# Black-Phoenix/CUDA-SfM

Hardware: AMD Instinct MI355X
Metric: RANSAC E-matrix hypotheses/sec (8-point, fused scoring), inlier-mask parity vs CPU oracle (higher is better)
Workload: dtype f32

## Files before the change

### cuda-sfm_amd/csrc/abi.hip

```cpp
#include "common.hpp"
#include "buffer_ranges.hpp"
#include "device_math.hpp"
#include "fuse_math.hpp"
#include "chain_adjust_math.hpp"
#include "ring_math.hpp"
#include <stdarg.h>
#include <stdio.h>
#include <string.h>
#include <new>
#include <atomic>
#include <vector>
#include <algorithm>
#include <initializer_list>

namespace sfm {

static thread_local char g_err[512] = "";

void set_error(const char *fmt, ...)
{
    va_list ap;
    va_start(ap, fmt);
    vsnprintf(g_err, sizeof(g_err), fmt, ap);
    va_end(ap);
// ... 494 lines not shown

int sfm_extract_sift(sfm_ctx *ctx, sfm_sift_point *d_sift, int max_pts, const float *d_image, int width, int height,
                     int pitch, int num_octaves, double init_blur, float thresh, float lowest_scale, int scale_up,
                     float *d_temp, int *num_pts, int *num_stored)
{
    SFM_REQUIRE(ctx && d_sift && d_image && num_pts, SFM_E_INVALID, "null argument");
    SFM_REQUIRE(width > 0 && height > 0 && width <= 16384 && height <= 16384 && pitch >= width, SFM_E_INVALID,
                "image %d x %d pitch %d", width, height, pitch);
    SFM_REQUIRE(num_octaves >= 1 && num_octaves <= 7, SFM_E_INVALID, "num_octaves %d outside 1..7", num_octaves);
    SFM_REQUIRE(max_pts > 0, SFM_E_INVALID, "max_pts %d", max_pts);
    *num_pts = 0;
    if (num_stored) *num_stored = 0;
    SFM_HIP_TRY(hipSetDevice(ctx->device));
    return launch_extract_sift(ctx, d_sift, max_pts, d_image, width, height, pitch, num_octaves, init_blur, thresh, lowest_scale,
                               scale_up ? 1 : 0, d_temp, num_pts, num_stored);
}

int sfm_extract_sift_begin(sfm_ctx *ctx, sfm_sift_point *d_sift, int max_pts, const float *d_image, int width, int height,
                           int pitch, int num_octaves, double init_blur, float thresh, float lowest_scale, int scale_up, float *d_temp)
{
    SFM_REQUIRE(ctx && d_sift && d_image, SFM_E_INVALID, "null argument");
    SFM_REQUIRE(width > 0 && height > 0 && width <= 16384 && height <= 16384 && pitch >= width, SFM_E_INVALID,
                "image %d x %d pitch %d", width, height, pitch);
    SFM_REQUIRE(num_octaves >= 1 && num_octaves <= 7, SFM_E_INVALID, "num_octaves %d outside 1..7", num_octaves);
    SFM_REQUIRE(max_pts > 0, SFM_E_INVALID, "max_pts %d", max_pts);
    SFM_HIP_TRY(hipSetDevice(ctx->device));
    return launch_extract_sift_begin(ctx, d_sift, max_pts, d_image, width, height, pitch, num_octaves, init_blur, thresh, lowest_scale,
                                     scale_up ? 1 : 0, d_temp);
}

int sfm_extract_sift_end(sfm_ctx *ctx, int *num_pts, int *num_stored)
{
    SFM_REQUIRE(ctx && num_pts, SFM_E_INVALID, "null argument");
    *num_pts = 0;
    if (num_stored) *num_stored = 0;
    SFM_HIP_TRY(hipSetDevice(ctx->device));
    return launch_extract_sift_end(ctx, num_pts, num_stored);
}

int sfm_find_homography(sfm_ctx *ctx, const sfm_sift_point *d_sift, int num_pts, float h_H[9], int *num_matches,
                        int num_loops, float min_score, float max_ambiguity, float thresh, uint32_t seed,
                        const int32_t *h_pts, int32_t *h_counts, float *h_homo)
{
    SFM_REQUIRE(ctx && h_H && num_matches, SFM_E_INVALID, "null argument");
    *num_matches = 0;
    for (int i = 0; i < 9; ++i) h_H[i] = (i % 4 == 0) ? 1.0f : 0.0f;
    if (!d_sift || num_pts < 8 || num_loops <= 0) return SFM_OK;
    SFM_HIP_TRY(hipSetDevice(ctx->device));
    const int L = round_up(num_loops, 16);
    if (h_pts) {
        for (size_t i = 0; i < (size_t)4 * L; ++i)
            SFM_REQUIRE(h_pts[i] >= 0 && h_pts[i] < num_pts, SFM_E_INVALID, "sample index %d out of range", h_pts[i]);
    }
    int num_valid = 0;
    return launch_homography(ctx, d_sift, num_pts, h_pts, L, thresh, min_score, max_ambiguity, seed, &num_valid, h_H, num_matches, h_counts, h_homo);
}

int sfm_pair_create(sfm_ctx *ctx, const float h_K[9], const float h_Kinv[9], int image_count, int num_points, sfm_pair **out)
{
    SFM_REQUIRE(out, SFM_E_INVALID, "null out pointer");
    *out = nullptr;
    SFM_REQUIRE(ctx && h_K && h_Kinv, SFM_E_INVALID, "null argument");
    SFM_REQUIRE(image_count == 2, SFM_E_INVALID, "image_count must be 2 (the reference only ever uses two views, sfm.h:31)");
    SFM_REQUIRE(num_points > 0, SFM_E_INVALID, "num_points must be positive");
    SFM_HIP_TRY(hipSetDevice(ctx->device));
    sfm_pair *p = new (std::nothrow) sfm_pair();
    SFM_REQUIRE(p, SFM_E_NOMEM, "host allocation failed");
    p->ctx = ctx;
    p->holds_ctx_ref = true; ctx->refs++;
    p->image_count = image_count;
    p->n = num_points;
    p->cap_points = num_points;
    p->ld = round_up(num_points, 128);
    memcpy(p->h_Kinv, h_Kinv, sizeof(p->h_Kinv));
    int rc = SFM_OK;
    auto A = [&](auto **ptr, size_t count) { if (rc == SFM_OK) rc = dev_alloc(ptr, count); };
    A(&p->d_K, 9); A(&p->d_Kinv, 9);
    for (int i = 0; i < 2; ++i) { A(&p->d_U[i], (size_t)3 * p->ld); A(&p->d_X[i], (size_t)3 * p->ld); }
    A(&p->d_pts4, (size_t)p->ld);
    A(&p->d_E, 9); A(&p->d_P, 64); A(&p->d_Pinv, 64); A(&p->d_Pind, 8);
    A(&p->d_points, (size_t)4 * num_points);
    A(&p->d_mask, (size_t)num_points);
    A(&p->slot[0].key, 2); A(&p->d_best, 2); A(&p->d_clk, kClkWords); A(&p->d_bound, 10);
    if (rc != SFM_OK) { sfm_pair_destroy(p); return rc; }
    hipError_t e = hipMemcpyAsync(p->d_K, h_K, 9 * sizeof(float), hipMemcpyHostToDevice, ctx->stream);
    if (e == hipSuccess) e = hipMemcpyAsync(p->d_Kinv, h_Kinv, 9 * sizeof(float), hipMemcpyHostToDevice, ctx->stream);
    if (e == hipSuccess) e = hipMemsetAsync(p->slot[0].key, 0, 2 * sizeof(unsigned long long), ctx->stream);
    p->state.key_clean = true;
    if (e == hipSuccess) e = hipMemsetAsync(p->d_best, 0, 2 * sizeof(uint32_t), ctx->stream);
    if (e == hipSuccess) e = hipMemsetAsync(p->d_bound, 0, 10 * sizeof(unsigned long long), ctx->stream);
    if (e == hipSuccess) e = hipMemsetAsync(p->d_clk, 0, kClkWords * sizeof(unsigned long long), ctx->stream);
    if (e == hipSuccess) e = hipMemsetAsync(p->d_Pind, 0, 8 * sizeof(int), ctx->stream);
    if (e == hipSuccess) e = hipStreamSynchronize(ctx->stream);
    if (e != hipSuccess) { sfm_pair_destroy(p); set_error("pair init failed: %s", hipGetErrorString(e)); return SFM_E_HIP; }
    *out = p;
    return SFM_OK;
}

int sfm_pair_reset(sfm_pair *pair, int num_points)
{
    SFM_REQUIRE(pair, SFM_E_INVALID, "null pair");
    SFM_FLUSH(pair);
    SFM_REQUIRE(num_points > 0 && num_points <= pair->cap_points, SFM_E_INVALID,
                "num_points %d outside (0, %d] (the size the pair was created with)", num_points, pair->cap_points);
    pair->n = num_points;
    pair->ld = round_up(num_points, 128);
    pair->state.reset();
    return SFM_OK;
}

int sfm_pair_destroy(sfm_pair *p)
{
    if (!p) return SFM_OK;
    if (p->ctx) { (void)hipSetDevice(p->ctx->device); (void)hipStreamSynchronize(p->ctx->stream); }
    void *bufs[] = { p->d_K, p->d_Kinv, p->d_U[0], p->d_U[1], p->d_X[0], p->d_X[1], p->d_pts4, p->d_E, p->d_P, p->d_Pinv, p->d_Pind,
                     p->d_points, p->d_mask, p->d_best, p->d_clk, p->d_bound, p->d_cells, p->d_pts4s, p->d_tile_boxes, p->d_buckets,
                     p->d_rstate, p->d_rpoints, p->d_rreproj, p->d_rwork, p->d_vstate, p->d_vreproj, p->d_vwork, p->d_vhyp, p->d_vcounts, p->d_awork,
                     p->d_lwork, p->d_lhyp };
    for (void *b : bufs) if (b) (void)hipFree(b);
    for (ShardSlot &s : p->slot) shard_slot_free(s);
    if (p->pipe_stream) { (void)hipStreamSynchronize(p->pipe_stream); (void)hipStreamDestroy(p->pipe_stream); }
    for (hipEvent_t e : p->pipe_final) if (e) (void)hipEventDestroy(e);
    if (p->pipe_call) (void)hipEventDestroy(p->pipe_call);
    if (p->cells_ev) (void)hipEventDestroy(p->cells_ev);
    if (p->pipe_keys) (void)hipFree(p->pipe_keys);
    sfm_ctx *owner = p->holds_ctx_ref ? p->ctx : nullptr;
    delete p;
    ctx_release(owner);
    return SFM_OK;
}

int sfm_fill_xu(sfm_pair *pair, const sfm_sift_point *d_data)
{
    SFM_REQUIRE(pair && d_data, SFM_E_INVALID, "null argument");
    SFM_FLUSH(pair);
    SFM_HIP_TRY(hipSetDevice(pair->ctx->device));
    const int rc = launch_fill_xu(pair, d_data);
    if (rc == SFM_OK) pair->state.points_filled(unit_z_Kinv(pair->h_Kinv));
    return rc;
}

int sfm_set_points(sfm_pair *pair, const float *d_X0, const float *d_X1)
{
    SFM_REQUIRE(pair && d_X0 && d_X1, SFM_E_INVALID, "null argument");
    SFM_FLUSH(pair);
    SFM_HIP_TRY(hipSetDevice(pair->ctx->device));
    const int rc = launch_set_points(pair, d_X0, d_X1);
    if (rc == SFM_OK) pair->state.points_set();
    return rc;
}

void sfm_ransac_default_params(sfm_ransac_params *p, int num_points)
{
    if (!p) return;
    memset(p, 0, sizeof(*p));
    p->num_hypotheses = num_points >= 8 ? (uint32_t)(num_points / 8) : 1u;
    p->seed = 0x5EED5F3Du;
    p->threshold = 1e-6f;
    p->jacobi_sweeps = 0;
    p->kernel = SFM_KERNEL_AUTO;
}

int sfm_ransac_permutation_indices(sfm_ctx *ctx, int num_points, uint32_t seed, int32_t *d_indices)
{
    SFM_REQUIRE(ctx && d_indices, SFM_E_INVALID, "null argument");
    SFM_REQUIRE(num_points >= 8, SFM_E_INVALID, "need at least 8 points");
    SFM_HIP_TRY(hipSetDevice(ctx->device));
    return launch_permutation_indices(ctx, num_points, seed, d_indices);
}

static int score_shard(sfm_pair *pair, const sfm_ransac_params *p, uint64_t *d_key_out, const float *d_E)
{
    uint32_t h0, count;
    int rc = resolve_shard(pair, p, &h0, &count);
    if (rc != SFM_OK) return rc;
    SFM_FLUSH(pair);
    SFM_HIP_TRY(hipSetDevice(pair->ctx->device));
    return launch_ransac_score(pair, pair->slot[0], pair->ctx->stream, *p, h0, count, reinterpret_cast<unsigned long long *>(d_key_out), d_E);
}

int sfm_ransac_score(sfm_pair *pair, const sfm_ransac_params *p) { return score_shard(pair, p, nullptr, nullptr); }

int sfm_ransac_score_candidates(sfm_pair *pair, const sfm_ransac_params *p, const float *d_E)
{
    SFM_REQUIRE(d_E, SFM_E_INVALID, "null candidate pointer");
    return score_shard(pair, p, nullptr, d_E);
}

int sfm_ransac_score_into(sfm_pair *pair, const sfm_ransac_params *p, uint64_t *d_key_out)
{
    SFM_REQUIRE(d_key_out, SFM_E_INVALID, "null key pointer");
    return score_shard(pair, p, d_key_out, nullptr);
}

int sfm_ransac_score_into_slot(sfm_pair *pair, const sfm_ransac_params *p, uint64_t *d_key_out, int slot, void *hip_stream)
{
    SFM_REQUIRE(d_key_out, SFM_E_INVALID, "null key pointer");
    SFM_REQUIRE(slot == 0 || slot == 1, SFM_E_INVALID, "slot must be 0 or 1");
    uint32_t h0, count;
// ... 1376 lines not shown
```

### cuda-sfm_amd/csrc/common.hpp

```cpp
#pragma once
#include <hip/hip_runtime.h>
#include <stdint.h>
#include <stddef.h>
#include <string>
#include <atomic>
#include <type_traits>
#include "../../include/sfm_amd.h"
#include "pair_state.hpp"
#include "job_order.hpp"
#if SFM_AB
#include "../../include/sfm_amd_ab.h"
#endif

#if SFM_AB
#define SFM_SW(p, i) ((p).reserved[i])
#else
#define SFM_SW(p, i) 0
#endif

namespace sfm {

void set_error(const char *fmt, ...);

#define SFM_HIP_TRY(expr)                                                                      \
    do {                                                                                       \
        hipError_t err__ = (expr);                                                             \
        if (err__ != hipSuccess) {                                                             \
            ::sfm::set_error("%s failed: %s (%s:%d)", #expr, hipGetErrorString(err__), __FILE__, __LINE__); \
            return err__ == hipErrorOutOfMemory ? SFM_E_NOMEM : SFM_E_HIP;                     \
        }                                                                                      \
    } while (0)

#define SFM_REQUIRE(cond, code, ...)                                                           \
    do {                                                                                       \
        if (!(cond)) { ::sfm::set_error(__VA_ARGS__); return (code); }                         \
    } while (0)

#define SFM_FLUSH(pair)                                                                        \
    do { if ((pair)->pipe_pending) { const int rcf__ = sfm_pair_flush(pair); if (rcf__ != SFM_OK) return rcf__; } } while (0)

#define SFM_NEED(pair, stages)                                                                 \
    SFM_REQUIRE((pair)->state.has(stages), SFM_E_STATE, "%s", ::sfm::pair_stage_hint((pair)->state.missing(stages)))

constexpr int kTraceBlocks = 1024;
constexpr int kTraceWords = 20;
constexpr int kClkWords = 8 + kTraceBlocks * kTraceWords;
inline int round_up(int v, int m) { return (v + m - 1) / m * m; }

template <typename T, typename N>
inline int grow(T **buf, N *have, size_t need, hipStream_t st)
{
    if (need <= (size_t)*have) return SFM_OK;
    SFM_HIP_TRY(hipStreamSynchronize(st));
    if (*buf) (void)hipFree(*buf);
    *buf = nullptr; *have = 0;
    SFM_HIP_TRY(hipMalloc(reinterpret_cast<void **>(buf), need * sizeof(std::conditional_t<std::is_void<T>::value, char, T>)));
    *have = (N)need;
    return SFM_OK;
}

inline bool unit_z_Kinv(const float h_Kinv[9]) { return h_Kinv[6] == 0.0f && h_Kinv[7] == 0.0f && h_Kinv[8] == 1.0f; }

struct Carver {
    uintptr_t base;
    size_t used = 0;
    explicit Carver(void *buffer) : base(reinterpret_cast<uintptr_t>(buffer)) {}
    template <typename T> T *take(size_t count, size_t align = 1)
    {
        used = (used + align - 1) & ~(align - 1);
        T *p = reinterpret_cast<T *>(base + used);
        used += count * sizeof(T);
        return p;
    }
};

struct JobArray {
    void *dev = nullptr, *pinned = nullptr;
    size_t cap = 0;
    hipEvent_t ev = nullptr;
};

inline int job_array_reserve(JobArray &j, size_t count, size_t elem, hipStream_t st)
{
    if (!j.ev) SFM_HIP_TRY(hipEventCreateWithFlags(&j.ev, hipEventDisableTiming));
    SFM_HIP_TRY(hipEventSynchronize(j.ev));
    if (count <= j.cap) return SFM_OK;
    const size_t want = count > 2 * j.cap ? count : 2 * j.cap;
    if (j.pinned) (void)hipHostFree(j.pinned);
    j.pinned = nullptr;
    j.cap = 0;
    SFM_HIP_TRY(hipHostMalloc(&j.pinned, want * elem, hipHostMallocDefault));
    size_t have = 0;
    const int rc = grow(&j.dev, &have, want * elem, st);
    if (rc != SFM_OK) return rc;
    j.cap = want;
    return SFM_OK;
}

inline int job_array_upload(JobArray &j, size_t count, size_t elem, hipStream_t st)
{
    SFM_HIP_TRY(hipMemcpyAsync(j.dev, j.pinned, count * elem, hipMemcpyHostToDevice, st));
    SFM_HIP_TRY(hipEventRecord(j.ev, st));
    return SFM_OK;
}

template <typename Job, typename Key, typename Fill>
inline int job_array_stage(JobArray &j, int count, hipStream_t st, Key key, Fill fill, const Job **d_jobs, int *largest)
{
    int rc = job_array_reserve(j, (size_t)count, sizeof(Job), st);
    if (rc != SFM_OK) return rc;
    const std::vector<int> order = order_by_decreasing_key(count, key);
    Job *h_jobs = static_cast<Job *>(j.pinned);
    for (int k = 0; k < count; ++k) fill(h_jobs[k], order[(size_t)k]);
    *d_jobs = static_cast<const Job *>(j.dev);
    *largest = key(order[0]);
    return job_array_upload(j, (size_t)count, sizeof(Job), st);
}

inline void job_array_free(JobArray &j)
{
    if (j.pinned) (void)hipHostFree(j.pinned);
    if (j.dev) (void)hipFree(j.dev);
    if (j.ev) (void)hipEventDestroy(j.ev);
    j = JobArray();
}

}

struct sfm_ctx {
// ... 28 lines not shown
    void *sift_temp = nullptr;
    size_t sift_temp_bytes = 0;
    void *sift_ws = nullptr;
    size_t sift_ws_bytes = 0;
    static constexpr int kPairLanes = 4;
    static constexpr int kViewLanes = 8;
    sfm_ctx *lane[kViewLanes - 1] = {};
    hipEvent_t lane_ev[kViewLanes] = {};
    sfm_pair *pool_pair = nullptr;
    float *views_pinned = nullptr, *views_image = nullptr;
    size_t views_floats = 0;
    hipEvent_t views_ev = nullptr;
    float pool_K[9] = {}, pool_Kinv[9] = {};
    float *pool_records = nullptr;
    size_t pool_records_cap = 0;
    void *batch_ws = nullptr;
    size_t batch_ws_bytes = 0;
    sfm::JobArray refine_jobs, register_jobs, view_points_jobs, adjust_jobs, align_jobs, fuse_jobs, chain_jobs, ring_jobs;
    void *fuse_ws = nullptr;
    size_t fuse_ws_bytes = 0;
    void *chain_ws = nullptr;
    size_t chain_ws_bytes = 0;
    void *ring_ws = nullptr;
    size_t ring_ws_bytes = 0;
    void *sift_job = nullptr;
    static constexpr int kBigLdsSlots = 16;
    const void *big_lds_done[kBigLdsSlots] = {};
};

inline int allow_big_lds(sfm_ctx *ctx, const void *kernel)
{
    for (int i = 0; i < sfm_ctx::kBigLdsSlots; ++i) {
        if (ctx->big_lds_done[i] == kernel) return SFM_OK;
        if (ctx->big_lds_done[i] == nullptr) {
            SFM_HIP_TRY(hipFuncSetAttribute(kernel, hipFuncAttributeMaxDynamicSharedMemorySize, 160 * 1024));
            ctx->big_lds_done[i] = kernel;
            return SFM_OK;
        }
    }
    SFM_HIP_TRY(hipFuncSetAttribute(kernel, hipFuncAttributeMaxDynamicSharedMemorySize, 160 * 1024));
    return SFM_OK;
}

struct ShardSlot {
    int *counts = nullptr;
    uint32_t *tick = nullptr;
    float *Ecand = nullptr;
    void *pf = nullptr;
    unsigned long long *key = nullptr;
    size_t cap_hyps = 0;
};

inline void shard_slot_free(ShardSlot &s)
{
    for (void *b : { (void *)s.counts, (void *)s.tick, (void *)s.Ecand, s.pf, (void *)s.key }) if (b) (void)hipFree(b);
    s = ShardSlot();
}

struct sfm_pair {
    sfm_ctx *ctx = nullptr;
    int image_count = 2;
    int n = 0;
    int cap_points = 0;
    int ld = 0;
    float *d_K = nullptr, *d_Kinv = nullptr;
    float *d_U[2] = { nullptr, nullptr };
    float *d_X[2] = { nullptr, nullptr };
    float4 *d_pts4 = nullptr;
    uint32_t sorted_epoch = 0;
    uint32_t pf_seen_epoch = 0;
    int pf_rule = 0;
    uint32_t *d_buckets = nullptr;
    size_t bucket_words = 0;
    uint32_t *d_tile_boxes = nullptr;
    int boxes_words = 0, boxes_tile = 0;
    float4 *d_pts4s = nullptr;
    float *d_E = nullptr;
    float *d_P = nullptr;
    float *d_Pinv = nullptr;
    int   *d_Pind = nullptr;
    float *d_points = nullptr;
    uint8_t *d_mask = nullptr;
    uint32_t *d_best = nullptr;
    unsigned long long *d_clk = nullptr;
    ShardSlot slot[2];
    unsigned long long *d_bound = nullptr;
    uint32_t bound_epoch = 0;
    uint32_t *d_cells = nullptr;
    hipEvent_t cells_ev = nullptr;
    hipStream_t cells_stream = nullptr;
    uint32_t cells_cap = 0, cells_mask = 0, cells_epoch = 0;
    uint32_t cand_h0 = 0, cand_seed = 0;
    const int32_t *cand_indices = nullptr;
    int cand_sweeps = 0;
    bool cand_given = false;
    hipStream_t pipe_stream = nullptr;
    hipEvent_t pipe_final[2] = { nullptr, nullptr }, pipe_call = nullptr;
    uint64_t *pipe_keys = nullptr;
    unsigned long long pipe_step = 0;
    bool pipe_pending = false;
    bool holds_ctx_ref = false;
    sfm::PairState state;
    float h_Kinv[9] = {};
    int pose_mode = SFM_POSE_REFERENCE;
    float *d_rstate = nullptr;
    float *d_rpoints = nullptr;
    float *d_rreproj = nullptr;
    void *d_rwork = nullptr;
    float *d_vstate = nullptr;
    float *d_vreproj = nullptr;
    void *d_vwork = nullptr;
    void *d_vhyp = nullptr;
    int *d_vcounts = nullptr;
    size_t cap_vhyps = 0;
    uint32_t view_hyps = 0;
    void *d_awork = nullptr;
    void *d_lwork = nullptr;
    void *d_lhyp = nullptr;
    size_t cap_lhyps = 0;
    int last_kernel = 0, last_grid = 0, last_block = 0, last_lds = 0;
};

namespace sfm {

int match_db_rows(const sfm_ctx *ctx, int n2);
int match_records(sfm_ctx *ctx, sfm_sift_point *d_sift1, int n1, const sfm_sift_point *d_sift2, int n2, int *out_idx);
int pose_chain(sfm_pair *pair, int mode, float *d_record);

int lane_contexts(sfm_ctx *ctx, int n, sfm_ctx **out);
int start_lanes_after(sfm_ctx *ctx, sfm_ctx *const *lanes, int n, hipEvent_t event);

int launch_ransac_score(sfm_pair *pair, ShardSlot &slot, hipStream_t stream, const sfm_ransac_params &p, uint32_t h0, uint32_t count,
                        unsigned long long *key2 = nullptr, const float *d_E_given = nullptr, bool serial = true);
int launch_ransac_finalize(sfm_pair *pair, const sfm_ransac_params &p, const unsigned long long *d_key, uint32_t hyp_host, bool from_key,
                           hipStream_t stream = nullptr, bool rederive = false);
int launch_permutation_indices(sfm_ctx *ctx, int n, uint32_t seed, int32_t *d_indices);
bool prefilter_usable(const sfm_pair *pair, const sfm_ransac_params &p, uint32_t count);
int prefilter_pick_rule(sfm_pair *pair, const sfm_ransac_params &p, uint32_t count);
int launch_score_prefilter(sfm_pair *pair, ShardSlot &slot, hipStream_t stream, const sfm_ransac_params &p, uint32_t h0, uint32_t count, unsigned long long *key2);
bool prefilter_sums_counts(const sfm_pair *pair, const sfm_ransac_params &p, uint32_t count);
int launch_pf_prep(sfm_pair *pair, ShardSlot &slot, hipStream_t stream, const sfm_ransac_params &p, uint32_t count);
int prefilter_tile_points(const sfm_pair *pair, const sfm_ransac_params &p);
int launch_pf_cells(sfm_pair *pair, hipStream_t stream, bool want_sorted = false, int tile = 0);
#if SFM_AB
int launch_score_prefilter_r2(sfm_pair *pair, ShardSlot &slot, hipStream_t stream, const sfm_ransac_params &p, uint32_t h0, uint32_t count, unsigned long long *key2);
int launch_score_mfma(sfm_pair *pair, ShardSlot &slot, hipStream_t stream, const sfm_ransac_params &p, uint32_t h0, uint32_t count);
int launch_prefilter_probe(sfm_ctx *ctx, const float *d_E, float thr, float B, const float pt[4], int survive_all, float *d_out);
int launch_prefilter_band_probe(sfm_ctx *ctx, const float *d_E, float thr, float B, const float box[8], int b_safe, const float pt[4], int survive_all, float *d_out);
#endif
int launch_ransac_fused(sfm_pair *pair, ShardSlot &slot, hipStream_t stream, const sfm_ransac_params &p, uint32_t h0, uint32_t count);
int launch_finalize_block(sfm_pair *pair, const sfm_ransac_params &p, const unsigned long long *d_key, uint32_t hyp_host, bool from_key,
                          hipStream_t stream, bool rederive);

int launch_fill_xu(sfm_pair *pair, const sfm_sift_point *d_data);
int launch_set_points(sfm_pair *pair, const float *d_X0, const float *d_X1);
int launch_pose_candidates(sfm_pair *pair, int mode);
int launch_choose_pose(sfm_pair *pair, int mode);
int launch_triangulate(sfm_pair *pair, int mode);
int launch_points_to_vbo(sfm_pair *pair, float *d_positions, float *d_velocities, float scale);
int launch_pair_record(sfm_pair *pair, int mode, float *d_record);
int launch_pose_chain(sfm_pair *pair, float *d_record);

int launch_refine(sfm_pair *pair, const sfm_refine_params &p);
int launch_refine_pairs(sfm_ctx *ctx, sfm_pair *const *pairs, int num_pairs, const sfm_refine_params &p, const uint8_t *const *d_masks);
size_t refine_work_bytes(int cap_points);
int refine_state_words();
// ... 85 lines not shown
```

### cuda-sfm_amd/csrc/ransac.hip

```cpp
#include "ransac_device.hpp"
#include "block_ops.hpp"
#include "prefilter_record.hpp"

namespace sfm {

__device__ __forceinline__ void reset_keys(unsigned long long *key, unsigned long long *key2)
{
    if (blockIdx.x == 0 && threadIdx.x == 0) {
        key[0] = 0ull; key[1] = 0ull;
        if (key2) *key2 = 0ull;
    }
}

template <int WPE>
__global__ __launch_bounds__(64, WPE)
void ransac_solve_lanes(const float *__restrict__ X0, const float *__restrict__ X1, int ld, int n,
                        const int32_t *__restrict__ indices, uint32_t seed, uint32_t h0, uint32_t count,
                        int sweeps, float *__restrict__ Ecand, unsigned long long *zero_key, unsigned long long *zero_key2,
                        int *__restrict__ zero_counts, uint32_t *__restrict__ zero_ticks, uint32_t nzero)
{
    reset_keys(zero_key, zero_key2);
    const uint32_t i = blockIdx.x * blockDim.x + threadIdx.x;
    if (zero_ticks) for (uint32_t w = i; w < nzero; w += gridDim.x * blockDim.x) zero_ticks[w] = 0u;
    if (i >= count) return;
// ... 142 lines not shown
    for (int t = t_first; t < t_last; ++t) {
        if (t > t_first) __syncthreads();
        if (threadIdx.x == 0) tile_bound = 0u;
        __syncthreads();
        const int first = t * tile;
        const float big = stage_tile<UNITZ>(lds, X0, X1, ld, first, min(tile, ld - first));
        atomicMax(&tile_bound, __float_as_uint(big));
        __syncthreads();
        const int nv = min(tile, n - first);
        const bool tame_tile = tile_bound < 0x47C35000u;
        for (uint32_t batch = blockIdx.x; batch < nbatch; batch += gridDim.x) {
            const uint32_t i = __builtin_amdgcn_readfirstlane((batch * WPB + wave) * NH);
            if (i >= count) continue;
            const int nh = (int)min((uint32_t)NH, count - i);
            Ess E[NH];
            bool e_tame = true;
#pragma unroll
            for (int h = 0; h < NH; ++h) {
                const float *e = Ecand + 9 * (size_t)(i + (h < nh ? h : 0));
                E[h] = Ess{ uniform(e[0]), uniform(e[1]), uniform(e[2]), uniform(e[3]), uniform(e[4]), uniform(e[5]), uniform(e[6]), uniform(e[7]), uniform(e[8]) };
                e_tame = e_tame && fabsf(E[h].e0) <= 2.0f && fabsf(E[h].e1) <= 2.0f && fabsf(E[h].e2) <= 2.0f && fabsf(E[h].e3) <= 2.0f &&
                         fabsf(E[h].e4) <= 2.0f && fabsf(E[h].e5) <= 2.0f && fabsf(E[h].e6) <= 2.0f && fabsf(E[h].e7) <= 2.0f && fabsf(E[h].e8) <= 2.0f;
            }
            int cnt[NH];
            if (NH > 1 && nh < NH) {
                const Ess e1[1] = { E[0] };
                int c1[1];
                if (e_tame && tame_tile) score_tile_n<UNITZ, false, 1>(e1, lds, nv, band, lane, c1);
                else score_tile_n<UNITZ, true, 1>(e1, lds, nv, band, lane, c1);
                cnt[0] = c1[0];
            } else if (e_tame && tame_tile) {
                score_tile_n<UNITZ, false, NH>(E, lds, nv, band, lane, cnt);
            } else {
                score_tile_n<UNITZ, true, NH>(E, lds, nv, band, lane, cnt);
            }
#pragma unroll
            for (int h = 0; h < NH; ++h) {
                if (h >= nh) break;
                int c = cnt[h];
                if (GRID2D) {
                    if (lane == 0 && c) atomicAdd(&counts[i + h], c);
                    continue;
                }
                if (ntiles > 1) {
                    int total = c;
                    if (lane == 0) {
                        if (t > 0) total += counts[i + h];
                        counts[i + h] = total;
                    }
                    c = __builtin_amdgcn_readfirstlane(total);
                } else if (lane == 0) {
                    counts[i + h] = c;
                }
                if (t == ntiles - 1) {
                    const unsigned long long key = pack_key((uint32_t)c, h0 + i + h);
                    wbest = key > wbest ? key : wbest;
                }
            }
        }
    }
    if (probe) { clk[0] = clock64() - c0; clk[1] = wall_clock64() - w0; }
    if (GRID2D) return;
    __syncthreads();
    unsigned long long *sbest = reinterpret_cast<unsigned long long *>(lds);
    if (lane == 0) sbest[wave] = wbest;
    __syncthreads();
    if (threadIdx.x == 0) {
        unsigned long long b = sbest[0];
#pragma unroll
        for (int w = 1; w < WPB; ++w) b = sbest[w] > b ? sbest[w] : b;
        if (b) {
            atomicMax(best_key, b);
            if (best_key2) atomicMax(best_key2, b);
        }
    }
}

__global__ __launch_bounds__(256)
void ransac_argmax_counts(const int *__restrict__ counts, uint32_t h0, uint32_t count,
                          unsigned long long *best_key, unsigned long long *best_key2)
{
    __shared__ unsigned long long sbest[4];
    unsigned long long b = 0;
    for (uint32_t i = blockIdx.x * blockDim.x + threadIdx.x; i < count; i += gridDim.x * blockDim.x) {
        const unsigned long long key = pack_key((uint32_t)counts[i], h0 + i);
        b = key > b ? key : b;
    }
    b = wave_max(b);
    if ((threadIdx.x & 63) == 0) sbest[threadIdx.x >> 6] = b;
    __syncthreads();
    if (threadIdx.x == 0) {
#pragma unroll
        for (int w = 1; w < 4; ++w) b = sbest[w] > b ? sbest[w] : b;
        if (b) {
            atomicMax(best_key, b);
            if (best_key2) atomicMax(best_key2, b);
        }
    }
}

static size_t tick_words(size_t count) { return 2 * count + 64; }

static int ensure_hyp_capacity(ShardSlot &s, hipStream_t stream, size_t count)
{
    if (count <= s.cap_hyps) return SFM_OK;
    SFM_HIP_TRY(hipStreamSynchronize(stream));
    for (void *b : { (void *)s.counts, (void *)s.Ecand, (void *)s.tick, s.pf }) if (b) (void)hipFree(b);
    s.counts = nullptr; s.Ecand = nullptr; s.tick = nullptr; s.pf = nullptr; s.cap_hyps = 0;
    SFM_HIP_TRY(hipMalloc(&s.tick, tick_words(count) * sizeof(uint32_t)));
    SFM_HIP_TRY(hipMalloc(&s.pf, count * sizeof(PfRecord)));
    SFM_HIP_TRY(hipMalloc(&s.counts, count * sizeof(int)));
    SFM_HIP_TRY(hipMalloc(&s.Ecand, count * 9 * sizeof(float)));
    s.cap_hyps = count;
    return SFM_OK;
}

static int launch_argmax_counts(const ShardSlot &s, hipStream_t stream, uint32_t h0, uint32_t count, unsigned long long *key2)
{
    const int ablocks = (int)((count + 4095u) / 4096u);
    hipLaunchKernelGGL(ransac_argmax_counts, dim3(ablocks < 1024 ? ablocks : 1024), dim3(256), 0, stream, s.counts, h0, count, s.key, key2);
    SFM_HIP_TRY(hipGetLastError());
    return SFM_OK;
}

template <int WPB, bool UNITZ, int NH = 1, bool GRID2D = false>
static int launch_score_t(sfm_pair *pair, ShardSlot &s, hipStream_t stream, uint32_t h0, uint32_t count, float thr, int tile, int ntiles, int grid, size_t lds, unsigned long long *key2)
{
    const int rc_lds = allow_big_lds(pair->ctx, reinterpret_cast<const void *>(&ransac_score_waves<WPB, UNITZ, NH, GRID2D>));
    if (rc_lds != SFM_OK) return rc_lds;
    hipLaunchKernelGGL((ransac_score_waves<WPB, UNITZ, NH, GRID2D>), dim3(grid, GRID2D ? ntiles : 1), dim3(WPB * 64), lds, stream,
                       pair->d_X[0], pair->d_X[1], pair->ld, pair->n, s.Ecand, h0, count, thr, tile, ntiles,
                       s.counts, s.key, key2, pair->d_clk);
    SFM_HIP_TRY(hipGetLastError());
    if (GRID2D) {
        const int rca = launch_argmax_counts(s, stream, h0, count, key2);
        if (rca != SFM_OK) return rca;
    }
    pair->last_grid = grid * (GRID2D ? ntiles : 1); pair->last_block = WPB * 64; pair->last_lds = (int)lds;
    return SFM_OK;
}

constexpr uint32_t kScalarSolveMax = 262144u;

int launch_ransac_score(sfm_pair *pair, ShardSlot &s, hipStream_t stream, const sfm_ransac_params &p, uint32_t h0, uint32_t count,
                        unsigned long long *key2, const float *d_E_given, bool serial)
{
    sfm_ctx *ctx = pair->ctx;
    const uint32_t fused_max = p.jacobi_sweeps > 0 ? 4096u : 1024u;
    int kernel = p.kernel == SFM_KERNEL_AUTO ? (count <= fused_max ? SFM_KERNEL_FUSED : SFM_KERNEL_SPLIT) : p.kernel;
    if (d_E_given && kernel == SFM_KERNEL_FUSED) kernel = SFM_KERNEL_SPLIT;
    const bool self_clearing = !d_E_given && count > 0 && (kernel == SFM_KERNEL_SPLIT || kernel == SFM_KERNEL_PREFILTER);
    if (!self_clearing) {
        if (!pair->state.key_clean) SFM_HIP_TRY(hipMemsetAsync(s.key, 0, 2 * sizeof(unsigned long long), stream));
        if (key2) SFM_HIP_TRY(hipMemsetAsync(key2, 0, sizeof(unsigned long long), stream));
    }
    pair->state.key_clean = false;
    pair->state.last_count = serial ? count : 0;
    pair->cand_given = serial && d_E_given != nullptr;
    if (serial) { pair->cand_h0 = h0; pair->cand_seed = p.seed; pair->cand_indices = p.d_indices; pair->cand_sweeps = p.jacobi_sweeps; }
    if (count == 0) return SFM_OK;
    int rc = ensure_hyp_capacity(s, stream, count);
    if (rc != SFM_OK) return rc;

#if SFM_AB
    if (kernel == SFM_KERNEL_MFMA && pair->n >= 65536) kernel = SFM_KERNEL_SPLIT;
#endif
    if (kernel == SFM_KERNEL_PREFILTER && !prefilter_usable(pair, p, 0x40000000u)) kernel = SFM_KERNEL_SPLIT;
    if (p.kernel == SFM_KERNEL_AUTO && kernel == SFM_KERNEL_SPLIT && prefilter_usable(pair, p, count) && SFM_SW(p, 3) != 1) kernel = SFM_KERNEL_PREFILTER;
    pair->last_kernel = kernel;
    if (kernel == SFM_KERNEL_FUSED) {
// ... 166 lines not shown
```

### cuda-sfm_amd/csrc/ransac_fused.hip

```cpp
#include "ransac_device.hpp"
#include "block_ops.hpp"
#include "pairs_batch.hpp"

namespace sfm {

constexpr int kWaveScratch = 256;

__device__ __forceinline__ void wave_sync()
{
    __builtin_amdgcn_fence(__ATOMIC_RELEASE, "wavefront");
    __builtin_amdgcn_wave_barrier();
    __builtin_amdgcn_fence(__ATOMIC_ACQUIRE, "wavefront");
}

__device__ __forceinline__ void tri_index(int lane, int &ei, int &ej)
{
    int e = lane < 45 ? lane : 0, i = 0;
    while (e >= 9 - i) { e -= 9 - i; ++i; }
    ei = i; ej = i + e;
}

__device__ __forceinline__ void build_jacobi_schedule(uint2 (*sched)[64], int lane)
{
    int ei, ej;
// ... 169 lines not shown
                if (staged) __syncthreads();
                const int first = t * tile;
                stage_tile<UNITZ>(lds, X0, X1, ld, first, min(tile, ld - first));
                __syncthreads();
                staged = true;
            }
            if (valid) cnt += score_tile<UNITZ>(E, lds, min(tile, n - t * tile), band, lane);
        }
        if (valid) {
            if (lane == 0) counts[i] = cnt;
            const unsigned long long key = pack_key((uint32_t)cnt, h0 + i);
            wbest = key > wbest ? key : wbest;
        }
    }
    __syncthreads();
    unsigned long long *sbest = reinterpret_cast<unsigned long long *>(lds);
    if (lane == 0) sbest[wave] = wbest;
    __syncthreads();
    if (threadIdx.x == 0) {
        unsigned long long b = sbest[0];
#pragma unroll
        for (int w = 1; w < WPB; ++w) b = sbest[w] > b ? sbest[w] : b;
        if (b) atomicMax(best_key, b);
    }
}

template <int WPB, bool UNITZ>
__global__ __launch_bounds__(WPB * 64)
void ransac_fused_waves(const float *__restrict__ X0, const float *__restrict__ X1, int ld, int n,
                        const int32_t *__restrict__ indices, uint32_t seed, int sweeps,
                        uint32_t h0, uint32_t count, float thr, int tile, int ntiles,
                        int *__restrict__ counts, float *__restrict__ Ecand, unsigned long long *best_key)
{
    extern __shared__ __attribute__((aligned(16))) float lds[];
    fused_body<WPB, UNITZ>(lds, X0, X1, ld, n, indices, seed, sweeps, h0, count, thr, tile, ntiles, counts, Ecand, best_key, blockIdx.x, gridDim.x);
}

__global__ __launch_bounds__(64)
void ransac_pairs_solve(const PairJob *__restrict__ jobs)
{
    const PairJob &j = jobs[blockIdx.y];
    const uint32_t i = blockIdx.x * 64u + threadIdx.x;
    if (i >= j.H) return;
    int idx[8];
    load_tuple(nullptr, j.seed, i, j.n, idx);
    float x1[8][3], x2[8][3];
#pragma unroll
    for (int k = 0; k < 8; ++k)
#pragma unroll
        for (int a = 0; a < 3; ++a) {
            x1[k][a] = j.X0[(size_t)a * j.ld + idx[k]];
            x2[k][a] = j.X1[(size_t)a * j.ld + idx[k]];
        }
    float E[9];
    nullvec9_householder(x1, x2, E);
    normalize_E(E);
#pragma unroll
    for (int k = 0; k < 9; ++k) j.Ecand[9 * (size_t)i + k] = E[k];
}

__global__ __launch_bounds__(8 * 64)
void ransac_fused_pairs(const PairJob *__restrict__ jobs)
{
    extern __shared__ __attribute__((aligned(16))) float lds[];
    const PairJob &j = jobs[blockIdx.y];
    const int tile = j.ld < kTileMax ? j.ld : kTileMax;
    const int ntiles = (j.ld + tile - 1) / tile;
    if ((uint32_t)blockIdx.x * 8u >= j.H) return;
    fused_body<8, true, true>(lds, j.X0, j.X1, j.ld, j.n, nullptr, j.seed, 0, 0u, j.H, j.thr, tile, ntiles, j.counts, j.Ecand, j.key, blockIdx.x, gridDim.x);
}

int launch_fused_pairs(sfm_ctx *ctx, const PairJob *d_jobs, int njobs, int blocks_per_pair, uint32_t max_H)
{
    const size_t lds = (size_t)2 * kUnitZSecond + (size_t)8 * kWaveScratch * sizeof(float) + 9 * 64 * sizeof(uint2);
    const int rc_lds = allow_big_lds(ctx, reinterpret_cast<const void *>(&ransac_fused_pairs));
    if (rc_lds != SFM_OK) return rc_lds;
    hipLaunchKernelGGL(ransac_pairs_solve, dim3((max_H + 63u) / 64u, njobs), dim3(64), 0, ctx->stream, d_jobs);
    SFM_HIP_TRY(hipGetLastError());
    hipLaunchKernelGGL(ransac_fused_pairs, dim3(blocks_per_pair, njobs), dim3(8 * 64), lds, ctx->stream, d_jobs);
    SFM_HIP_TRY(hipGetLastError());
    return SFM_OK;
}

__global__ __launch_bounds__(1024)
void ransac_finalize_block(const float *__restrict__ X0, const float *__restrict__ X1, int ld, int n,
                           const int32_t *__restrict__ indices, uint32_t seed, int sweeps,
                           const unsigned long long *__restrict__ key, uint32_t hyp_host, int from_key,
                           const float *__restrict__ Ecand, uint32_t h0, uint32_t count, uint32_t num_hypotheses,
                           float thr, float *__restrict__ E_out, uint8_t *__restrict__ mask, uint32_t *__restrict__ best_out)
{
    __shared__ __attribute__((aligned(16))) float ws[kWaveScratch];
    __shared__ uint2 sched[9][64];
    __shared__ float sE[9];
    __shared__ int scount[16];
    uint32_t hyp = hyp_host;
    if (from_key) hyp = 0xFFFFFFFFu - (uint32_t)(key[0] & 0xFFFFFFFFull);
    hyp = __builtin_amdgcn_readfirstlane(hyp);
    if (hyp >= num_hypotheses) {
        if (threadIdx.x < 9) E_out[threadIdx.x] = 0.0f;
        if (threadIdx.x == 0) { best_out[0] = 0xFFFFFFFFu; best_out[1] = 0; }
        for (int j = threadIdx.x; j < n; j += blockDim.x) mask[j] = 0;
        return;
    }
    if (threadIdx.x < 64) {
        if (Ecand && hyp >= h0 && hyp - h0 < count) {
            if (threadIdx.x < 9) sE[threadIdx.x] = Ecand[9 * (size_t)(hyp - h0) + threadIdx.x];
        } else {
            float E[9];
            if (sweeps > 0) build_jacobi_schedule(sched, threadIdx.x);
            wave_sync();
            solve_wave(X0, X1, ld, n, indices, seed, hyp, sweeps, ws, sched, threadIdx.x, E);
            if (threadIdx.x == 0) {
#pragma unroll
                for (int k = 0; k < 9; ++k) sE[k] = E[k];
            }
        }
    }
    __syncthreads();
    if (threadIdx.x < 9) E_out[threadIdx.x] = sE[threadIdx.x];
    const Ess E{ sE[0], sE[1], sE[2], sE[3], sE[4], sE[5], sE[6], sE[7], sE[8] };
    int c = 0;
    for (int j0 = 0; j0 < n; j0 += blockDim.x) {
        const int j = j0 + threadIdx.x;
        bool in = false;
        if (j < n) {
            const float r = residual(E, X0[j], X0[(size_t)ld + j], X0[2 * (size_t)ld + j],
                                     X1[j], X1[(size_t)ld + j], X1[2 * (size_t)ld + j]);
            in = r < thr;
            mask[j] = in ? 1 : 0;
        }
        c += __builtin_popcountll(__ballot(in));
    }
    if ((threadIdx.x & 63) == 0) scount[threadIdx.x >> 6] = c;
    __syncthreads();
    if (threadIdx.x == 0) {
        int total = 0;
#pragma unroll
        for (int w = 0; w < 16; ++w) total += scount[w];
        best_out[0] = hyp;
        best_out[1] = (uint32_t)total;
    }
}

template <int WPB, bool UNITZ>
static int launch_fused_t(sfm_pair *pair, ShardSlot &s, hipStream_t stream, const sfm_ransac_params &p, uint32_t h0, uint32_t count, int tile, int ntiles, int grid, size_t lds)
{
    const int rc_lds = allow_big_lds(pair->ctx, reinterpret_cast<const void *>(&ransac_fused_waves<WPB, UNITZ>));
    if (rc_lds != SFM_OK) return rc_lds;
    hipLaunchKernelGGL((ransac_fused_waves<WPB, UNITZ>), dim3(grid), dim3(WPB * 64), lds, stream,
                       pair->d_X[0], pair->d_X[1], pair->ld, pair->n, p.d_indices, p.seed, p.jacobi_sweeps,
                       h0, count, p.threshold, tile, ntiles, s.counts, s.Ecand, s.key);
    SFM_HIP_TRY(hipGetLastError());
    pair->last_grid = grid; pair->last_block = WPB * 64; pair->last_lds = (int)lds;
    return SFM_OK;
}

int launch_ransac_fused(sfm_pair *pair, ShardSlot &s, hipStream_t stream, const sfm_ransac_params &p, uint32_t h0, uint32_t count)
{
    sfm_ctx *ctx = pair->ctx;
    const int tile = pair->ld < kTileMax ? pair->ld : kTileMax;
    const int ntiles = (pair->ld + tile - 1) / tile;
    int wpb = 8;
    while (wpb > 4 && (count + wpb - 1) / wpb < (uint32_t)ctx->num_cus) wpb >>= 1;
    const uint32_t nbatch = (count + wpb - 1) / wpb;
    const int grid = (int)(nbatch < (uint32_t)ctx->num_cus ? nbatch : (uint32_t)ctx->num_cus);
    const bool uz = pair->state.unit_z;
    const size_t lds = (uz ? (size_t)2 * kUnitZSecond : (size_t)6 * tile * sizeof(float)) + (size_t)wpb * kWaveScratch * sizeof(float) +
                       9 * 64 * sizeof(uint2);
    const bool timed = ctx->timing && ctx->tcount < sfm_ctx::kTimingSlots;
    hipEvent_t *tev = timed ? ctx->tev[ctx->tcount] : nullptr;
    if (timed) { SFM_HIP_TRY(hipEventRecord(tev[0], stream)); SFM_HIP_TRY(hipEventRecord(tev[1], stream)); }
    int rc;
    switch (wpb) {
    case 8:  rc = uz ? launch_fused_t<8, true>(pair, s, stream, p, h0, count, tile, ntiles, grid, lds) : launch_fused_t<8, false>(pair, s, stream, p, h0, count, tile, ntiles, grid, lds); break;
    default: rc = uz ? launch_fused_t<4, true>(pair, s, stream, p, h0, count, tile, ntiles, grid, lds) : launch_fused_t<4, false>(pair, s, stream, p, h0, count, tile, ntiles, grid, lds); break;
    }
    if (rc == SFM_OK && timed) { SFM_HIP_TRY(hipEventRecord(tev[2], stream)); ctx->tcount++; }
    return rc;
}

int launch_finalize_block(sfm_pair *pair, const sfm_ransac_params &p, const unsigned long long *d_key,
                          uint32_t hyp_host, bool from_key, hipStream_t stream, bool rederive)
{
    const bool cand_ok = !rederive && pair->state.last_count > 0 && pair->cand_seed == p.seed && pair->cand_indices == p.d_indices &&
                         pair->cand_sweeps == p.jacobi_sweeps;
    hipLaunchKernelGGL(ransac_finalize_block, dim3(1), dim3(1024), 0, stream,
                       pair->d_X[0], pair->d_X[1], pair->ld, pair->n, p.d_indices, p.seed, p.jacobi_sweeps,
                       d_key, hyp_host, from_key ? 1 : 0,
                       cand_ok ? pair->slot[0].Ecand : nullptr, pair->cand_h0, pair->state.last_count, p.num_hypotheses,
                       p.threshold, pair->d_E, pair->d_mask, pair->d_best);
    SFM_HIP_TRY(hipGetLastError());
    return SFM_OK;
}

}
```

### profiles/exchange_trace.py

```python
import csv
import glob
import json
import os
import sys

ROOT = os.path.dirname(os.path.dirname(os.path.abspath(__file__)))
sys.path.insert(0, ROOT)


def run():
    import numpy as np
    import torch
    import cuda_sfm_amd as S
    from cuda_sfm_amd import synth
    sys.path.insert(0, os.path.join(ROOT, "tests"))
    dev = torch.device("cuda", 0)
    n, H = 4096, 131072
    scene = synth.two_view_scene(n)
    ctx = S.Context(0, torch.cuda.current_stream().cuda_stream)
    pair = S.ImagePair(ctx, scene["K"], scene["Kinv"], 2, n)
    pair.fillXU(torch.from_numpy(scene["sift"].view(np.uint8).reshape(n, 576)).to(dev))
    comm = S.Comm(ctx, S.Comm.unique_id(), 0, 1)
    p = S.default_params(n, num_hypotheses=H)
    for k in range(10):
        p.seed = 100 + k
        comm.estimate_E_pipelined(pair, p)
    comm.flush(); torch.cuda.synchronize()
    torch.cuda.nvtx.range_push("pipelined_exchange") if hasattr(torch.cuda, "nvtx") else None
    for k in range(40):
        p.seed = 200 + k
        comm.estimate_E_pipelined(pair, p)
    comm.flush(); torch.cuda.synchronize()
    hyp, cnt = pair.get_best()
    print(json.dumps({"part": 1, "steps": 40, "best": [hyp, cnt], "nccl_ranks": comm.nccl_ranks()}), flush=True)
    from helpers import read_pnm_grey
    dino = os.path.join(ROOT, "tests", "golden", "dino")
    names = sorted(f for f in os.listdir(dino) if f.startswith("dino_grey_"))[:6]
    images = [read_pnm_grey(os.path.join(dino, f)) for f in names]
    pairs = [(i, j) for i in range(len(images)) for j in range(i + 1, len(images))]
    K = np.float32([[2360, 0, 360], [0, 2360, 288], [0, 0, 1]]); Kinv = np.linalg.inv(K.astype(np.float64)).astype(np.float32)
    res, counts = comm.process_views(images, K, Kinv, pairs=pairs, max_pts=4096)
    torch.cuda.synchronize()
    print(json.dumps({"part": 2, "views": len(images), "pairs": len(res), "features": counts, "exchange": comm.last_exchange()}), flush=True)
    comm.close()


def load(d, suffix):
    rows = []
    for f in glob.glob(os.path.join(d, "**", "*" + suffix), recursive=True):
        rows += list(csv.DictReader(open(f)))
    return rows


def report(d):
    kern = load(d, "kernel_trace.csv")
    api = load(d, "hip_api_trace.csv")
    mem = load(d, "memory_copy_trace.csv")
    ks = sorted(((int(r["Start_Timestamp"]), int(r["End_Timestamp"]), r["Kernel_Name"].split("(")[0].replace("void ", ""), r.get("Queue_Id", "?"), r.get("Stream_Id", "?")) for r in kern))
    print(f"{len(ks)} kernel records, {len(api)} HIP API records, {len(mem)} memory copies")
    by_name = {}
    for s, e, nme, q, st in ks:
        by_name.setdefault(nme, []).append((s, e, q, st))
    for nme, v in sorted(by_name.items(), key=lambda kv: -len(kv[1]))[:12]:
        qs = sorted({x[2] for x in v}); sts = sorted({x[3] for x in v})
        print(f"  {len(v):5d} x {nme[:70]:70s} queues {qs} streams {sts} avg {sum(e - s for s, e, _, _ in v) / len(v) / 1e3:.1f} us")
    fin = [x for x in by_name.get("sfm::ransac_finalize_block", [])]
    score = [x for nme, v in by_name.items() if "ransac_score_prefilter" in nme for x in v]
    solve = [x for nme, v in by_name.items() if "ransac_solve_lanes1_qr" in nme for x in v]
    rccl = [x for nme, v in by_name.items() if "nccl" in nme.lower() for x in v]
    compute = sorted(score + solve)
    fin = sorted(fin)[-45:-5] if len(fin) >= 45 else sorted(fin)
    ov = []
    for s, e, q, st in fin:
        o = sum(max(0, min(e, ce) - max(s, cs)) for cs, ce, cq, cst in compute if (cq, cst) != (q, st))
        ov.append((e - s, o))
    if ov:
        full = sum(1 for d_, o in ov if o >= 0.9 * d_)
        print(f"part 1: {len(ov)} finalize launches on the exchange stream: mean duration {sum(d_ for d_, _ in ov) / len(ov) / 1e3:.2f} us, "
              f"mean time overlapped by solve / scoring kernels of OTHER queues {sum(o for _, o in ov) / len(ov) / 1e3:.2f} us; "
              f"{full} of {len(ov)} run entirely under the next step's kernels")
        print(f"        finalize queue / stream ids {sorted({(q, st) for _, _, q, st in fin})}; scoring {sorted({(q, st) for _, _, q, st in score})}; solve {sorted({(q, st) for _, _, q, st in solve})}")
    print(f"        RCCL kernels in the trace: {len(rccl)} (a one-rank all-reduce of 8 bytes in place is a no-op or a copy: {len(mem)} memory copies)")
    rapi = sorted(load(d, "rccl_api_trace.csv"), key=lambda r: int(r["Start_Timestamp"]))
    calls = {}
    for r in rapi:
        calls[r["Function"]] = calls.get(r["Function"], 0) + 1
    print(f"part 2: RCCL API calls: {dict(sorted(calls.items()))}")
    syncs = sorted((int(r["Start_Timestamp"]), int(r["End_Timestamp"]), r["Function"], r.get("Thread_Id")) for r in api
                   if r["Function"] in ("hipStreamSynchronize", "hipDeviceSynchronize", "hipEventSynchronize"))
    groups, open_t = [], {}
    for r in rapi:
        tid = r.get("Thread_Id")
        if r["Function"] == "ncclGroupStart":
            open_t[tid] = [int(r["Start_Timestamp"]), 0, 0]
        elif r["Function"] == "ncclBroadcast" and tid in open_t:
            open_t[tid][2] += 1
        elif r["Function"] == "ncclGroupEnd" and tid in open_t:
            g = open_t.pop(tid); g[1] = int(r["End_Timestamp"]); groups.append((g[0], g[1], g[2], tid))
    worst = 0
    for g0, g1, nb, tid in groups:
        inside = [s_ for s_ in syncs if g0 <= s_[0] <= g1 and s_[3] == tid]
        worst = max(worst, len(inside))
    nb_all = [g[2] for g in groups]
    print(f"        {len(groups)} ncclGroupStart..ncclGroupEnd groups, broadcasts per group {sorted(set(nb_all))}, longest group {max((g[1] - g[0]) for g in groups) / 1e3 if groups else 0:.1f} us; "
          f"host synchronisations of the calling thread INSIDE a group: {worst} at most; {len(syncs)} host synchronisations in the whole run")
    allred = [r for r in rapi if r["Function"] == "ncclAllReduce"]
    if allred:
        dur = [int(r["End_Timestamp"]) - int(r["Start_Timestamp"]) for r in allred]
        print(f"        ncclAllReduce: {len(allred)} calls, host-side enqueue {sum(dur) / len(dur) / 1e3:.1f} us on average (max {max(dur) / 1e3:.1f})")


if __name__ == "__main__":
    if sys.argv[1:2] == ["run"]:
        run()
    else:
        report(sys.argv[2] if len(sys.argv) > 2 else ".")
```

Before: 2.892 billion.

## Split RANSAC finalize across wave-sized blocks with atomic last-block reduction

```diff
diff --git a/cuda-sfm_amd/csrc/abi.hip b/cuda-sfm_amd/csrc/abi.hip
--- a/cuda-sfm_amd/csrc/abi.hip
+++ b/cuda-sfm_amd/csrc/abi.hip
@@ -600,12 +600,14 @@
     A(&p->d_points, (size_t)4 * num_points);
     A(&p->d_mask, (size_t)num_points);
     A(&p->slot[0].key, 2); A(&p->d_best, 2); A(&p->d_clk, kClkWords); A(&p->d_bound, 10);
+    A(&p->d_fin, kFinalWords);
     if (rc != SFM_OK) { sfm_pair_destroy(p); return rc; }
     hipError_t e = hipMemcpyAsync(p->d_K, h_K, 9 * sizeof(float), hipMemcpyHostToDevice, ctx->stream);
     if (e == hipSuccess) e = hipMemcpyAsync(p->d_Kinv, h_Kinv, 9 * sizeof(float), hipMemcpyHostToDevice, ctx->stream);
     if (e == hipSuccess) e = hipMemsetAsync(p->slot[0].key, 0, 2 * sizeof(unsigned long long), ctx->stream);
     p->state.key_clean = true;
     if (e == hipSuccess) e = hipMemsetAsync(p->d_best, 0, 2 * sizeof(uint32_t), ctx->stream);
+    if (e == hipSuccess) e = hipMemsetAsync(p->d_fin, 0, kFinalWords * sizeof(uint32_t), ctx->stream);
     if (e == hipSuccess) e = hipMemsetAsync(p->d_bound, 0, 10 * sizeof(unsigned long long), ctx->stream);
     if (e == hipSuccess) e = hipMemsetAsync(p->d_clk, 0, kClkWords * sizeof(unsigned long long), ctx->stream);
     if (e == hipSuccess) e = hipMemsetAsync(p->d_Pind, 0, 8 * sizeof(int), ctx->stream);
@@ -632,7 +634,7 @@
     if (!p) return SFM_OK;
     if (p->ctx) { (void)hipSetDevice(p->ctx->device); (void)hipStreamSynchronize(p->ctx->stream); }
     void *bufs[] = { p->d_K, p->d_Kinv, p->d_U[0], p->d_U[1], p->d_X[0], p->d_X[1], p->d_pts4, p->d_E, p->d_P, p->d_Pinv, p->d_Pind,
-                     p->d_points, p->d_mask, p->d_best, p->d_clk, p->d_bound, p->d_cells, p->d_pts4s, p->d_tile_boxes, p->d_buckets,
+                     p->d_points, p->d_mask, p->d_best, p->d_fin, p->d_clk, p->d_bound, p->d_cells, p->d_pts4s, p->d_tile_boxes, p->d_buckets,
                      p->d_rstate, p->d_rpoints, p->d_rreproj, p->d_rwork, p->d_vstate, p->d_vreproj, p->d_vwork, p->d_vhyp, p->d_vcounts, p->d_awork,
                      p->d_lwork, p->d_lhyp };
     for (void *b : bufs) if (b) (void)hipFree(b);
diff --git a/cuda-sfm_amd/csrc/common.hpp b/cuda-sfm_amd/csrc/common.hpp
--- a/cuda-sfm_amd/csrc/common.hpp
+++ b/cuda-sfm_amd/csrc/common.hpp
@@ -45,6 +45,7 @@
 constexpr int kTraceBlocks = 1024;
 constexpr int kTraceWords = 20;
 constexpr int kClkWords = 8 + kTraceBlocks * kTraceWords;
+constexpr int kFinalWords = 65;
 inline int round_up(int v, int m) { return (v + m - 1) / m * m; }
 
 template <typename T, typename N>
@@ -239,6 +240,7 @@
     float *d_points = nullptr;
     uint8_t *d_mask = nullptr;
     uint32_t *d_best = nullptr;
+    uint32_t *d_fin = nullptr;
     unsigned long long *d_clk = nullptr;
     ShardSlot slot[2];
     unsigned long long *d_bound = nullptr;
diff --git a/cuda-sfm_amd/csrc/ransac.hip b/cuda-sfm_amd/csrc/ransac.hip
--- a/cuda-sfm_amd/csrc/ransac.hip
+++ b/cuda-sfm_amd/csrc/ransac.hip
@@ -248,10 +248,23 @@
 {
     __shared__ unsigned long long sbest[4];
     unsigned long long b = 0;
-    for (uint32_t i = blockIdx.x * blockDim.x + threadIdx.x; i < count; i += gridDim.x * blockDim.x) {
-        const unsigned long long key = pack_key((uint32_t)counts[i], h0 + i);
+    const auto fold = [&](int c, uint32_t i) {
+        const unsigned long long key = pack_key((uint32_t)c, h0 + i);
         b = key > b ? key : b;
-    }
+    };
+    const uint32_t tid = blockIdx.x * blockDim.x + threadIdx.x, nthreads = gridDim.x * blockDim.x;
+    const uint32_t to_boundary = (4u - (uint32_t)((reinterpret_cast<uintptr_t>(counts) >> 2) & 3u)) & 3u;
+    const uint32_t head = to_boundary < count ? to_boundary : count;
+    const uint32_t nvec = (count - head) >> 2, tail = head + 4u * nvec;
+    if (tid < head) fold(counts[tid], tid);
+    const int4 *__restrict__ body = reinterpret_cast<const int4 *>(counts + head);
+#pragma unroll 4
+    for (uint32_t q = tid; q < nvec; q += nthreads) {
+        const int4 c = body[q];
+        const uint32_t i = head + 4u * q;
+        fold(c.x, i); fold(c.y, i + 1u); fold(c.z, i + 2u); fold(c.w, i + 3u);
+    }
+    if (tid < count - tail) fold(counts[tail + tid], tail + tid);
     b = wave_max(b);
     if ((threadIdx.x & 63) == 0) sbest[threadIdx.x >> 6] = b;
     __syncthreads();
diff --git a/cuda-sfm_amd/csrc/ransac_fused.hip b/cuda-sfm_amd/csrc/ransac_fused.hip
--- a/cuda-sfm_amd/csrc/ransac_fused.hip
+++ b/cuda-sfm_amd/csrc/ransac_fused.hip
@@ -275,63 +275,77 @@
     return SFM_OK;
 }
 
-__global__ __launch_bounds__(1024)
-void ransac_finalize_block(const float *__restrict__ X0, const float *__restrict__ X1, int ld, int n,
+constexpr int kFinalSlice = 256;
+constexpr int kFinalMaxBlocks = 64;
+
+template <bool JACOBI>
+__global__ __launch_bounds__(64, JACOBI ? 4 : 5)
+void ransac_finalize_waves(const float *__restrict__ X0, const float *__restrict__ X1, int ld, int n,
                            const int32_t *__restrict__ indices, uint32_t seed, int sweeps,
                            const unsigned long long *__restrict__ key, uint32_t hyp_host, int from_key,
                            const float *__restrict__ Ecand, uint32_t h0, uint32_t count, uint32_t num_hypotheses,
-                           float thr, float *__restrict__ E_out, uint8_t *__restrict__ mask, uint32_t *__restrict__ best_out)
+                           float thr, float *__restrict__ E_out, uint8_t *__restrict__ mask, uint32_t *__restrict__ best_out,
+                           uint32_t *__restrict__ fin)
 {
     __shared__ __attribute__((aligned(16))) float ws[kWaveScratch];
-    __shared__ uint2 sched[9][64];
-    __shared__ float sE[9];
-    __shared__ int scount[16];
+    __shared__ uint2 sched[JACOBI ? 9 : 1][64];
+    const int lane = threadIdx.x;
     uint32_t hyp = hyp_host;
     if (from_key) hyp = 0xFFFFFFFFu - (uint32_t)(key[0] & 0xFFFFFFFFull);
     hyp = __builtin_amdgcn_readfirstlane(hyp);
-    if (hyp >= num_hypotheses) {
-        if (threadIdx.x < 9) E_out[threadIdx.x] = 0.0f;
-        if (threadIdx.x == 0) { best_out[0] = 0xFFFFFFFFu; best_out[1] = 0; }
-        for (int j = threadIdx.x; j < n; j += blockDim.x) mask[j] = 0;
-        return;
-    }
-    if (threadIdx.x < 64) {
+    const bool winner = hyp < num_hypotheses;
+    float e[9] = { 0, 0, 0, 0, 0, 0, 0, 0, 0 };
+    if (winner) {
         if (Ecand && hyp >= h0 && hyp - h0 < count) {
-            if (threadIdx.x < 9) sE[threadIdx.x] = Ecand[9 * (size_t)(hyp - h0) + threadIdx.x];
+#pragma unroll
+            for (int k = 0; k < 9; ++k) e[k] = Ecand[9 * (size_t)(hyp - h0) + k];
         } else {
-            float E[9];
-            if (sweeps > 0) build_jacobi_schedule(sched, threadIdx.x);
-            wave_sync();
-            solve_wave(X0, X1, ld, n, indices, seed, hyp, sweeps, ws, sched, threadIdx.x, E);
-            if (threadIdx.x == 0) {
-#pragma unroll
-                for (int k = 0; k < 9; ++k) sE[k] = E[k];
+            if (JACOBI) { build_jacobi_schedule(sched, lane); wave_sync(); }
+            __builtin_assume(!JACOBI || sweeps > 0);
+            solve_wave(X0, X1, ld, n, indices, seed, hyp, JACOBI ? sweeps : 0, ws, sched, lane, e);
+        }
+    }
+    if (blockIdx.x == 0 && lane < 9) {
+        float v = e[0];
+#pragma unroll
+        for (int k = 1; k < 9; ++k) v = (lane == k) ? e[k] : v;
+        E_out[lane] = v;
+    }
+    const Ess E{ uniform(e[0]), uniform(e[1]), uniform(e[2]), uniform(e[3]), uniform(e[4]), uniform(e[5]), uniform(e[6]), uniform(e[7]), uniform(e[8]) };
+    int c = 0;
+    for (int base = (int)blockIdx.x * kFinalSlice; base < n; base += (int)gridDim.x * kFinalSlice) {
+#pragma unroll
+        for (int q = 0; q < kFinalSlice / 64; ++q) {
+            const int j = base + 64 * q + lane;
+            bool in = false;
+            if (j < n) {
+                if (winner) {
+                    const float r = residual(E, X0[j], X0[(size_t)ld + j], X0[2 * (size_t)ld + j],
+                                             X1[j], X1[(size_t)ld + j], X1[2 * (size_t)ld + j]);
+                    in = r < thr;
+                }
+                mask[j] = in ? 1 : 0;
             }
-        }
-    }
-    __syncthreads();
-    if (threadIdx.x < 9) E_out[threadIdx.x] = sE[threadIdx.x];
-    const Ess E{ sE[0], sE[1], sE[2], sE[3], sE[4], sE[5], sE[6], sE[7], sE[8] };
-    int c = 0;
-    for (int j0 = 0; j0 < n; j0 += blockDim.x) {
-        const int j = j0 + threadIdx.x;
-        bool in = false;
-        if (j < n) {
-            const float r = residual(E, X0[j], X0[(size_t)ld + j], X0[2 * (size_t)ld + j],
-                                     X1[j], X1[(size_t)ld + j], X1[2 * (size_t)ld + j]);
-            in = r < thr;
-            mask[j] = in ? 1 : 0;
-        }
-        c += __builtin_popcountll(__ballot(in));
-    }
-    if ((threadIdx.x & 63) == 0) scount[threadIdx.x >> 6] = c;
-    __syncthreads();
-    if (threadIdx.x == 0) {
-        int total = 0;
-#pragma unroll
-        for (int w = 0; w < 16; ++w) total += scount[w];
-        best_out[0] = hyp;
-        best_out[1] = (uint32_t)total;
+            c += __builtin_popcountll(__ballot(in));
+        }
+    }
+    const uint32_t nblocks = gridDim.x;
+    uint32_t t = 0;
+    if (lane == 0) {
+        __hip_atomic_store(&fin[blockIdx.x], (uint32_t)c, __ATOMIC_RELAXED, __HIP_MEMORY_SCOPE_AGENT);
+        t = __hip_atomic_fetch_add(&fin[kFinalMaxBlocks], 1u, __ATOMIC_ACQ_REL, __HIP_MEMORY_SCOPE_AGENT);
+    }
+    t = __builtin_amdgcn_readfirstlane(t);
+    if (t != nblocks - 1) return;
+    __builtin_amdgcn_fence(__ATOMIC_ACQUIRE, "agent");
+    uint32_t part = 0;
+    if ((uint32_t)lane < nblocks) part = __hip_atomic_load(&fin[lane], __ATOMIC_RELAXED, __HIP_MEMORY_SCOPE_AGENT);
+    uint32_t total = 0;
+    for (uint32_t b = 0; b < nblocks; ++b) total += (uint32_t)__shfl((int)part, (int)b);
+    if (lane == 0) {
+        best_out[0] = winner ? hyp : 0xFFFFFFFFu;
+        best_out[1] = total;
+        __hip_atomic_store(&fin[kFinalMaxBlocks], 0u, __ATOMIC_RELAXED, __HIP_MEMORY_SCOPE_AGENT);
     }
 }
 
@@ -377,11 +391,15 @@
 {
     const bool cand_ok = !rederive && pair->state.last_count > 0 && pair->cand_seed == p.seed && pair->cand_indices == p.d_indices &&
                          pair->cand_sweeps == p.jacobi_sweeps;
-    hipLaunchKernelGGL(ransac_finalize_block, dim3(1), dim3(1024), 0, stream,
+    const int slices = (pair->n + kFinalSlice - 1) / kFinalSlice;
+    const dim3 grid(slices < kFinalMaxBlocks ? slices : kFinalMaxBlocks);
+    static_assert(kFinalMaxBlocks + 1 <= kFinalWords && kFinalMaxBlocks <= 64, "partials + ticket fit the pair's scratch; one lane reads one partial");
+    const auto kernel = p.jacobi_sweeps > 0 ? &ransac_finalize_waves<true> : &ransac_finalize_waves<false>;
+    hipLaunchKernelGGL(kernel, grid, dim3(64), 0, stream,
                        pair->d_X[0], pair->d_X[1], pair->ld, pair->n, p.d_indices, p.seed, p.jacobi_sweeps,
                        d_key, hyp_host, from_key ? 1 : 0,
                        cand_ok ? pair->slot[0].Ecand : nullptr, pair->cand_h0, pair->state.last_count, p.num_hypotheses,
-                       p.threshold, pair->d_E, pair->d_mask, pair->d_best);
+                       p.threshold, pair->d_E, pair->d_mask, pair->d_best, pair->d_fin);
     SFM_HIP_TRY(hipGetLastError());
     return SFM_OK;
 }
diff --git a/profiles/exchange_trace.py b/profiles/exchange_trace.py
--- a/profiles/exchange_trace.py
+++ b/profiles/exchange_trace.py
@@ -64,7 +64,7 @@
     for nme, v in sorted(by_name.items(), key=lambda kv: -len(kv[1]))[:12]:
         qs = sorted({x[2] for x in v}); sts = sorted({x[3] for x in v})
         print(f"  {len(v):5d} x {nme[:70]:70s} queues {qs} streams {sts} avg {sum(e - s for s, e, _, _ in v) / len(v) / 1e3:.1f} us")
-    fin = [x for x in by_name.get("sfm::ransac_finalize_block", [])]
+    fin = [x for nme, v in by_name.items() if "ransac_finalize_" in nme for x in v]
     score = [x for nme, v in by_name.items() if "ransac_score_prefilter" in nme for x in v]
     solve = [x for nme, v in by_name.items() if "ransac_solve_lanes1_qr" in nme for x in v]
     rccl = [x for nme, v in by_name.items() if "nccl" in nme.lower() for x in v]
```

After: 2.890 billion. No clear change (-0.1%).
